# Dfam-consortium/RepeatAfterMe

Measured on AMD Instinct MI355X. Metric: flank_bp_aligned_per_sec (extension columns/s x flanks), higher is better.
Workload: dtype int32

## Files before the change

repeatafterme_amd/csrc/ramx_device.hip:

```cpp

#include <rccl/rccl.h>
#include <errno.h>
#include <fcntl.h>
#include <limits.h>
#include <sys/mman.h>
#include <unistd.h>
#include <stdarg.h>
#include <stdio.h>
#include <stdlib.h>
#include <string.h>
#include <time.h>
#include <algorithm>
#include <memory>
#include <vector>

#include "ramx_kernels_common.h"
#include "ramx_kernels_stream.h"
#include "ramx_kernels_resident.h"
#include "ramx_cp_api.h"
#include "ramx_pk_api.h"
#include "ramx_profile_api.h"
#include "ramx_align_api.h"
#include "ramx_pileup_api.h"
#include "ramx_dinuc_api.h"
// ... 774 lines not shown

static int direction_route(ramx_dev *d, const KArgs &a, int L, DirRoute *out)
{
  const RouteEnv e = route_env();
  DirRoute rt = route_gates(e, a.W, a.go, a.ge, a.tab, L, d->Nx, d->pk_r0, d->cp_flanks_ok != 0, d->trace_cb != NULL || d->verbose_cb != NULL,
                            dev_is_multi(d), d->peer_ready != 0, d->nranks, d->force_chain != 0, d->cus);
  const int W = a.W, tiles = d->Np / 64;
  if (rt.int32_can)
  {
    const int rc = (W == 14) ? prk_plan<14>(tiles, d->cus, &rt.block, &rt.blocks) : (W == 20) ? prk_plan<20>(tiles, d->cus, &rt.block, &rt.blocks) :
                   (W == 40) ? prk_plan<40>(tiles, d->cus, &rt.block, &rt.blocks) : prk_plan<80>(tiles, d->cus, &rt.block, &rt.blocks);
    if (rc != RAMX_OK) return rc;
  }
  if (rt.pk && ramx_pk_shape(W, tiles, &rt.pk_block, &rt.pk_blocks) != RAMX_OK) { ramx_set_error("packed-row kernel: occupancy query failed"); return RAMX_ERR_HIP; }
  route_settle(rt, e, d->Nx);
  *out = rt;
  return RAMX_OK;
}

static int mailbox_clear(ramx_dev *d)
{
  if (!d->hostbox_host) HIPCHK(hipMemsetAsync(d->xbox, 0, sizeof(PeerBox), d->stream));
  HIPCHK(hipStreamSynchronize(d->stream));
  if (d->hostbox_host) { memset((void *)d->hostbox_host, 0, sizeof(PeerBox)); __sync_synchronize(); }
  return RAMX_OK;
}

static int mailbox_mirror(ramx_dev *d, PeerBox **mirror)
{
  *mirror = NULL;
  if (!d->hostbox_host) return RAMX_OK;
  if (!d->hostbox_mirror) HIPCHK(hipMalloc((void **)&d->hostbox_mirror, sizeof(PeerBox)));
  HIPCHK(hipMemsetAsync(d->hostbox_mirror, 0, sizeof(PeerBox), d->stream));
  *mirror = d->hostbox_mirror;
  return RAMX_OK;
}

static int read_launch_state(ramx_dev *d, RamxCtl c[2], unsigned *errw)
{
  unsigned long long ew = 0;
  HIPCHK(hipStreamSynchronize(d->stream));
  int rc = d2h_small(d, c, d->d_ctl, 2 * sizeof(RamxCtl));
  if (rc == RAMX_OK) rc = d2h_small(d, &ew, d->d_err, sizeof(ew));
  *errw = (unsigned)ew;
  return rc;
}

#ifdef RAMX_PRK_TIMING
static int prk_timing_report(ramx_dev *d, unsigned long long *dbgbuf, size_t nw, bool pk, int block, int blocks, int L, int pk_r0)
{
  HIPCHK(hipStreamSynchronize(d->stream));
  unsigned long long *h = (unsigned long long *)malloc(nw * 8 * sizeof(unsigned long long));
  HIPCHK(hipMemcpy(h, dbgbuf, nw * 8 * sizeof(unsigned long long), hipMemcpyDeviceToHost));
  static const char *nm[6] = { "wait vote", "block barrier 1", "band", pk ? "early arrival" : "reduce+barrier 2", pk ? "late arrival" : "issue atomics", "loop top" };
  const int wpb = block / 64;
  fprintf(stderr, "PRK_TIMING %s blocks %d x %d threads, L %d, first row %d (ns per column)\n", pk ? "packed rows" : "int32 rows", blocks, block, L, pk ? pk_r0 : 0);
  for (int k = 0; k < 6; k++)
  {
    double s0 = 0, sO = 0, mx = 0, mn = 1e30;
    for (size_t i = 0; i < nw; i++)
    {
      const double v = 10.0 * (double)h[i * 8 + k] / L;
      if ((int)(i % wpb) == 0) s0 += v; else sO += v;
      if (v > mx) mx = v;
      if (v < mn) mn = v;
    }
    fprintf(stderr, "PRK_TIMING %-18s wave0 avg %8.1f  other waves avg %8.1f  min %8.1f  max %8.1f\n", nm[k], s0 / blocks,
            wpb > 1 ? sO / (double)(nw - blocks) : 0.0, mn, mx);
  }
  fprintf(stderr, "PRK_TIMING band by wave index:");
  for (int wv = 0; wv < wpb; wv++)
  {
    double sw = 0;
    for (int b = 0; b < blocks - 1; b++) sw += 10.0 * (double)h[((size_t)b * wpb + wv) * 8 + 2] / L;
    fprintf(stderr, " w%d %.0f", wv, sw / (blocks > 1 ? blocks - 1 : 1));
  }
  fprintf(stderr, "\n");
  {
    int gb = 0;
    for (int b = 1; b < blocks; b++) if (h[(size_t)b * wpb * 8 + 0] < h[(size_t)gb * wpb * 8 + 0]) gb = b;
    fprintf(stderr, "PRK_TIMING workgroup %d (shortest vote wait), per wave: wait vote | barrier | band | early | late | top\n", gb);
    for (int wv = 0; wv < wpb; wv++)
    {
      const unsigned long long *q = h + ((size_t)gb * wpb + wv) * 8;
      fprintf(stderr, "PRK_TIMING   w%d %7.0f %7.0f %7.0f %7.0f %7.0f %7.0f   rows full %llu lean %llu\n", wv, 10.0 * q[0] / L, 10.0 * q[1] / L, 10.0 * q[2] / L,
              10.0 * q[3] / L, 10.0 * q[4] / L, 10.0 * q[5] / L, q[6], q[7]);
    }
  }
  {
    const double half = L - L / 2;
    size_t never = 0, always = 0, wg_any = 0;
    double lanes = 0, cols = 0;
    int hist[6] = { 0, 0, 0, 0, 0, 0 };
    for (int b = 0; b < blocks; b++)
    {
      bool any = false;
      for (int wv = 0; wv < wpb; wv++)
      {
        const size_t i = (size_t)b * wpb + wv;
        const double c = (double)h[i * 8 + 6], l = (double)h[i * 8 + 7];
        if (c == 0) { never++; continue; }
        any = any || c > 0.5 * half;
        if (c > 0.9 * half) always++;
        lanes += l; cols += c;
        const double avg = l / c;
        hist[avg <= 1 ? 0 : avg <= 2 ? 1 : avg <= 4 ? 2 : avg <= 8 ? 3 : avg <= 16 ? 4 : 5]++;
      }
      if (any) wg_any++;
    }
    fprintf(stderr, "PRK_LEANSTAT second half (%.0f columns): %zu of %zu waves always LEAN, %zu non-LEAN in > 90 %% of the columns; workgroups with a wave "
            "non-LEAN in > 50 %%: %zu of %d; lanes per non-LEAN wave-column %.2f; waves by that average <=1: %d <=2: %d <=4: %d <=8: %d <=16: %d more: %d\n",
            half, never, nw, always, wg_any, blocks, cols > 0 ? lanes / cols : 0.0, hist[0], hist[1], hist[2], hist[3], hist[4], hist[5]);
  }
  free(h);
  (void)hipFree(dbgbuf);
  return RAMX_OK;
}

static int fam_timing_report(const unsigned long long *dbg)
{
  unsigned long long h[64];
  HIPCHK(hipMemcpy(h, dbg, sizeof(h), hipMemcpyDeviceToHost));
  static const char *nm[6] = { "vote + stop rule", "winner table+barrier", "band + contrib", "wave reduce", "end barrier", "loop top" };
  const double cols = h[6] ? (double)h[6] : 1.0;
  fprintf(stderr, "FAM_TIMING family 0 (block 0), %.0f columns, ns per column per wave:\n", cols);
  for (int k = 0; k < 6; k++)
    fprintf(stderr, "FAM_TIMING %-22s w0 %7.1f  w1 %7.1f  w2 %7.1f  w3 %7.1f\n", nm[k], 10.0 * h[k] / cols, 10.0 * h[8 + k] / cols,
            10.0 * h[16 + k] / cols, 10.0 * h[24 + k] / cols);
  return RAMX_OK;
}
#endif

#ifdef RAMX_CP_TIMING
static int cp_family_timing_report(const unsigned long long *dbg)
{
  unsigned long long h[16 * 16 + 8];
  HIPCHK(hipMemcpy(h, dbg, sizeof(h), hipMemcpyDeviceToHost));
  static const char *nm[12] = { "vote read + stop rule", "(after speculative band)", "row update", "reductions", "records/slide/window",
                                "sum+atomics+barrier", "-", "loop top", "wait: drain", "wait: samples + polling", "wait: fold",
                                "wait: LDS + barrier" };
  const double cols = h[16 * 16] ? (double)h[16 * 16] : 1.0;
  fprintf(stderr, "CP_TIMING block 0, %.0f columns, shader clocks per column (waves 0, 1, last two):\n", cols);
  int nw = 0;
  for (int w = 0; w < 16; w++) if (h[w * 16 + 0]) nw = w + 1;
  for (int k = 0; k < 12; k++)
    if (k == 6) fprintf(stderr, "CP_TIMING mispredicted columns: %.0f of %.0f\n", (double)h[6], cols);
    else fprintf(stderr, "CP_TIMING %-24s w0 %7.1f  w1 %7.1f  w%d %7.1f  w%d %7.1f\n", nm[k], h[k] / cols, h[16 + k] / cols,
                        nw > 1 ? nw - 2 : 0, h[(nw > 1 ? nw - 2 : 0) * 16 + k] / cols, nw > 0 ? nw - 1 : 0, h[(nw > 0 ? nw - 1 : 0) * 16 + k] / cols);
  return RAMX_OK;
}
#endif

static int prk_run(ramx_dev *d, const KArgs &a, int L, DirRoute &rt, bool *used)
{
  *used = false;
  const int W = a.W;
  const bool multi = rt.multi;
  int rc;
  if (multi)
  {
    int cannot = rt.int32_can ? 0 : 1;
    if ((rc = host_allreduce_flag(d, &cannot)) != RAMX_OK) return rc;
    rt.int32_can = !cannot;
  }
  const bool pk = rt.pk;
  const int pk_r0 = rt.pk_r0, pk_block = rt.pk_block, pk_blocks = rt.pk_blocks;
  int block = rt.block, blocks = rt.blocks;
// ... 18 lines not shown
  }
  memcpy(pa.tab, a.tab, sizeof(pa.tab));
  pa.pack_ok = getenv("RAMX_NO_FASTPACK") ? 0 : fast_pack_ok(pa.tab, a.go, a.ge, L, W);
  if (pa.pack_ok && getenv("RAMX_NO_MASKHI") == NULL) pa.pack_ok = 2;
  pa.lean_p = lean_p_of(pa.tab, a.go, a.ge);
  { const char *lm = getenv("RAMX_LEADER_MAX"); pa.leader_max = lm ? atoi(lm) : 3; if (pa.leader_max < 0) pa.leader_max = 0; if (pa.leader_max > 64) pa.leader_max = 64; }
  PKArgs ka;
  memset(&ka, 0, sizeof(ka));
  ka.spread = rt.spread; ka.rebase = rt.rebase;
  if (!pk && (rc = pack_rest(d)) != RAMX_OK) return rc;
  HIPCHK(hipMemsetAsync(d->d_vote, 0, PRK_NSETS * NSHARD * sizeof(PShard), d->stream));
  HIPCHK(hipMemsetAsync(d->d_err, 0, 64, d->stream));
  long long *sums_next = d->d_sums + (size_t)NSHARD * 4;
  const bool head = !pk || pk_r0 > 0;
  if (pk && pk_r0 > 0) { pa.L = pk_r0; pa.sums_next = sums_next; }
#ifdef RAMX_PRK_TIMING
  const size_t nw = pk ? (size_t)pk_blocks * (pk_block / 64) : (size_t)blocks * (block / 64);
  unsigned long long *dbgbuf = NULL;
  HIPCHK(hipMalloc((void **)&dbgbuf, nw * 8 * sizeof(unsigned long long)));
  HIPCHK(hipMemset(dbgbuf, 0, nw * 8 * sizeof(unsigned long long)));
  if (pk) ka.dbg = dbgbuf; else pa.dbg = dbgbuf;
#endif
  rc = RAMX_OK;
  const bool tmarks = getenv("RAMX_TIMING") != NULL;
  const double tm0 = now_ms();
  rt_mark("persistent route, memsets");
  if (head)
  {
    if (block == 256)
      rc = (W == 14) ? prk_launch<14, 256>(d, pa, blocks) : (W == 20) ? prk_launch<20, 256>(d, pa, blocks) :
           (W == 40) ? prk_launch<40, 256>(d, pa, blocks) : prk_launch<80, 256>(d, pa, blocks);
    else
      rc = (W == 14) ? prk_launch<14, 512>(d, pa, blocks) : (W == 20) ? prk_launch<20, 512>(d, pa, blocks) : prk_launch<40, 512>(d, pa, blocks);
  }
  rt_mark("first rows launched (int32 kernel)");
  if (rc == RAMX_OK && pk)
  {
    ka.S = d->d_state[0]; ka.bases = d->d_bases; ka.bounds = d->d_bounds; ka.trim = d->d_trim;
    ka.vote = d->d_vote; ka.cons_out = d->d_cons; ka.err = d->d_err;
    ka.peers = pa.peers; ka.box = pa.box; ka.mirror = pa.mirror; ka.rank = pa.rank; ka.nranks = pa.nranks;
    ka.xblock = 0;
    if (ka.nranks > 1 && getenv("RAMX_NO_PK_EXCHANGER") == NULL)
    {
      int cap = 0;
      if (ramx_pk_capacity(W, pk_block, &cap) == RAMX_OK && pk_blocks + 1 <= cap) ka.xblock = pk_blocks;
    }
    ka.Np = d->Np; ka.Nx = d->Nx; ka.L = L; ka.go = a.go; ka.ge = a.ge; ka.cap = a.cap; ka.minimp = a.minimp;
    ka.when_to_stop = a.when_to_stop; ka.nblocks = pk_blocks;
    memcpy(ka.tab, a.tab, sizeof(ka.tab));
    ka.lean_p = pa.lean_p; ka.leader_max = pa.leader_max;
    ka.spec_on = getenv("RAMX_NO_PK_SPEC") == NULL ? 1 : 0;
    { const char *we = getenv("RAMX_TEST_PK_WRONG_EVERY"); ka.test_wrong_every = we ? atoi(we) : 0; }
    { const char *ck = getenv("RAMX_PK_CKPT"); const int v = ck ? atoi(ck) : 0; ka.ckpt = (v == 1 || v == 2 || v == 4 || v == 8) ? v : 0; }
    { const char *ts = getenv("RAMX_TEST_PK_SPREAD"); if (ts) ka.spread = atoi(ts); }
    ka.spread_rows = ka.spread;
    { const char *ts = getenv("RAMX_TEST_PK_SPREAD_ROWS"); if (ts) ka.spread_rows = atoi(ts); }
    d->last_packed_r0 = pk_r0;
    const int seg = pk_segment_columns(L, a.when_to_stop);
    const int NWw = (2 * W + 1 + 8) / 8 + 2;
    long long *sbuf[2] = { d->d_sums + (size_t)NSHARD * 4, d->d_sums + (size_t)2 * NSHARD * 4 };
    const long long *sums_in = pk_r0 > 0 ? sbuf[0] : d->d_sums;
    int nextbuf = pk_r0 > 0 ? 1 : 0;
    int ctl_i = 0;
    auto words_for = [&](int r_end) { int wn = ((r_end + 7) >> 3) + NWw + 2; return wn < d->KW ? wn : d->KW; };
    if (ka.nranks > 1 && !head) test_delay_rank(d);
    for (int r = pk_r0, s_i = 0; r < L && rc == RAMX_OK; s_i++)
    {
      const int r1 = seg > 0 ? std::min(L, (r / seg + 1) * seg) : L;
      if ((rc = pack_settle(d)) != RAMX_OK) return rc;
      if (d->packed_kw < words_for(r1))
      {
        if ((rc = launch_pack(d, d->Nx, d->Np, W, d->packed_kw, words_for(r1), d->stream)) != RAMX_OK) break;
        d->packed_kw = words_for(r1);
      }
      HIPCHK(hipMemsetAsync(d->d_vote, 0, PRK_NSETS * NSHARD * sizeof(PShard), d->stream));
      ka.r0 = r; ka.Lseg = r1; ka.sums_in = sums_in;
      ka.sums_next = r1 < L ? sbuf[nextbuf] : NULL;
      if (r1 < L) HIPCHK(hipMemsetAsync(sbuf[nextbuf], 0, (size_t)NSHARD * 4 * sizeof(long long), d->stream));
      ka.ctl_in = d->d_ctl + ctl_i; ka.ctl_out = d->d_ctl + (ctl_i ^ 1);
      if (r == 0) ka.ctl_out = d->d_ctl;
      const double tm1 = now_ms();
      rc = ramx_pk_launch(d->stream, W, pk_block, pk_blocks, ka);
      if (rc != RAMX_OK) { ramx_set_error("packed-row kernel: launch failed (W %d, %d workgroups of %d threads)", W, pk_blocks, pk_block); break; }
      if (tmarks) fprintf(stderr, "RAMX_TIMING       run: piece %d (rows %d..%d, %d x %d threads) launched %.3f ms after the first launch (launch call %.3f ms)\n", s_i, r, r1, pk_blocks, pk_block, now_ms() - tm0, now_ms() - tm1);
      const int out_i = (r == 0) ? 0 : (ctl_i ^ 1);
      if (r1 >= L) break;
      const int r2 = std::min(L, (r1 / seg + 1) * seg);
      if (d->packed_kw < words_for(r2))
      {
        if ((rc = launch_pack(d, d->Nx, d->Np, W, d->packed_kw, words_for(r2), d->pack_stream)) != RAMX_OK) break;
        HIPCHK(hipEventRecord(d->pack_done, d->pack_stream));
        d->pack_busy = 1;
        d->packed_kw = words_for(r2);
      }
      RamxCtl c2[2];
      unsigned errw = 0;
      HIPCHK(hipStreamSynchronize(d->stream));
      if (tmarks) fprintf(stderr, "RAMX_TIMING       run: piece %d complete %.3f ms after the first launch\n", s_i, now_ms() - tm0);
      if ((rc = read_launch_state(d, c2, &errw)) != RAMX_OK) break;
      rt_mark("piece: control block and error word read");
      const RamxCtl &hc = c2[out_i];
      if (hc.stopped || hc.pad != 0 || errw != 0 || hc.rows_done < r1) break;
      sums_in = sbuf[nextbuf]; nextbuf ^= 1; ctl_i = out_i; r = r1;
    }
    if (pk) { block = pk_block; blocks = pk_blocks; }
  }
// ... 2317 lines not shown
```

repeatafterme_amd/csrc/ramx_kernels_packed.h:

```cpp
#pragma once

#include "ramx_kernels_vote.h"
#include "ramx_pk_api.h"

template <int W>
struct PkCfg
{
  static constexpr int B = 2 * W + 1, NP = W + 1, NW = (B + 8) / 8 + 2, NG = (B + 31) / 32, Q = W + 1;
};

#define PKB_NEG2 ((int)0x80008000u)
#ifndef PKB_GROUP
#define PKB_GROUP 2
#endif
#ifndef PKB_PT
#define PKB_PT 2
#endif

__device__ __forceinline__ int pkb_add_sat(int a, int b) { return pk_i(__builtin_elementwise_add_sat(pk_v(a), pk_v(b))); }
__device__ __forceinline__ int pkb_sub_sat(int a, int b) { return pk_i(__builtin_elementwise_sub_sat(pk_v(a), pk_v(b))); }
__device__ __forceinline__ int pkb_max(int a, int b) { return pk_i(__builtin_elementwise_max(pk_v(a), pk_v(b))); }
__device__ __forceinline__ void pkb_add_to_hi(int &dst, int a, int b) { asm("v_add_i16 %0, %1, %2 op_sel:[0,0,1] clamp" : "+v"(dst) : "v"(a), "v"(b)); }
__device__ __forceinline__ int pkb_add_lo(int a, int b) { int d; asm("v_add_i16 %0, %1, %2 clamp" : "=v"(d) : "v"(a), "v"(b)); return d; }
__device__ __forceinline__ int pkb_hmax(int p) { const pk_s2 q = pk_v(p); return q.x > q.y ? (int)q.x : (int)q.y; }
__device__ __forceinline__ unsigned pkb_lds_off(const void *p) { return (unsigned)(size_t)(__attribute__((address_space(3))) const void *)p; }

__device__ __forceinline__ unsigned pkb_mask_word(unsigned wv, int kb, int bdy9x4 )
{
  int s = bdy9x4 - 32 * kb;
  s = s < 0 ? 0 : s;
  const unsigned m = s >= 32 ? 0u : (0xffffffffu << s);
  return wv | m;
}

struct PkTabs
{
  int4 t4[4][256];
  int tp[4][256];
};

template <int BLOCK>
__device__ __forceinline__ void pkb_tabs_init(PkTabs &pt, const int (&tab)[RAMX_NCLASS][4])
{
  for (int i = threadIdx.x; i < 256; i += BLOCK)
  {
    const int hi = i >> 4, lo = (i & 15) ^ ((hi & 3) << 2);
    int q[4];
#pragma unroll
    for (int c = 0; c < 4; c++)
    {
      const int sl = lo < RAMX_NCLASS ? tab[lo][c] : (lo == 15 ? -32768 : 0);
      const int sh = hi < RAMX_NCLASS ? tab[hi][c] : (hi == 15 ? -32768 : 0);
      q[c] = (sl & 0xffff) | (sh << 16);
      pt.tp[c][i] = q[c];
    }
#pragma unroll
    for (int wv = 0; wv < 4; wv++) pt.t4[wv][i] = make_int4(q[wv], q[(wv + 1) & 3], q[(wv + 2) & 3], q[(wv + 3) & 3]);
  }
}

template <int W, int BLOCK, bool FULL>
__device__ __forceinline__ void pkb_band(const int go2, const int ge2, const PkTabs &pt, const int wsel, const int ph4, const unsigned (&w)[PkCfg<W>::NW],
                                         int (&R)[PkCfg<W>::NP], int (&E)[PkCfg<W>::NP], int &best, int (&kg)[PkCfg<W>::NG], int (&bA)[4], int &maxE)
{
// ... 143 lines not shown
    if (hit[h]) jb = 64 * h + __builtin_ctzll(hit[h]);
  if (lane == leader)
  {
#pragma unroll
    for (int c = 0; c < 4; c++) bestA[c] = best[c];
    jbest = jb;
  }
}

template <class A>
__device__ __forceinline__ int pkb_stop_rule(const A &a, const int r, const long long (&v)[4], const int fl, int *st, const int lane)
{
  long long mx = ((long long)__builtin_amdgcn_readfirstlane(st[1]) << 32) | (long long)(unsigned)__builtin_amdgcn_readfirstlane(st[0]);
  int mr = __builtin_amdgcn_readfirstlane(st[2]), ov = __builtin_amdgcn_readfirstlane(st[3]);
  long long cw = 0;
  int bw = 0;
#pragma unroll
  for (int k = 0; k < 4; k++)
  {
    const long long vk = ((long long)__builtin_amdgcn_readfirstlane((int)(v[k] >> 32)) << 32) |
                         (long long)(unsigned)__builtin_amdgcn_readfirstlane((int)v[k]);
    if (vk > 2147483647LL || vk < -2147483648LL) ov = 1;
    if (vk > cw) { cw = vk; bw = k; }
  }
  int dist = mr - r;
  dist = dist < 0 ? -dist : dist;
  const int nm = cw >= mx + (long long)dist * a.minimp ? 1 : 0;
  if (nm && !fl) { mr = r; mx = cw; }
  int d2 = r - mr;
  d2 = d2 < 0 ? -d2 : d2;
  const int stp = d2 >= a.when_to_stop ? 1 : 0;
  if (lane == 0) { st[0] = (int)mx; st[1] = (int)(mx >> 32); st[2] = mr; st[3] = ov; }
  return bw | (nm << 2) | (stp << 3) | (fl << 4);
}

#ifdef RAMX_PRK_TIMING
#ifdef RAMX_PRK_TIMING_TAIL
#define PKB_TICK_ON (2 * r >= a.L)
#else
#define PKB_TICK_ON true
#endif
#define PKB_TICK(k) do { const unsigned long long t_ = wall_clock64(); if (PKB_TICK_ON) tsum[k] += t_ - tlast; tlast = t_; } while (0)
#else
#define PKB_TICK(k) do { } while (0)
#endif

template <int W, int BLOCK>
__global__ __launch_bounds__(BLOCK, BLOCK / 256) void ramx_packed_kernel(const PKArgs a)
{
  constexpr int NP = PkCfg<W>::NP, NW = PkCfg<W>::NW, NG = PkCfg<W>::NG, Q = PkCfg<W>::Q, WPB = BLOCK / 64;
  constexpr bool VW = (BLOCK % 256) != 0;
  constexpr int BW = VW ? WPB - 1 : WPB, VOTER = VW ? BW : 0;
  constexpr bool SPEC = W <= 40;
  struct Smem
  {
    PkTabs pt;
    long long tot[2][2][4];
    int word[2][2];
    int cnt[2][2];
    int st[4];
    int lead[WPB][2 * NP + NW + 1];
    int eb[SPEC ? BLOCK * NP : 1];
  };
  __shared__ __attribute__((aligned(16))) Smem sm;
  const int lane = threadIdx.x & 63, wave = threadIdx.x >> 6;
  const int tile = blockIdx.x * BW + wave;
  const bool live = wave < BW && tile < (a.Np >> 6);
  const int n = (live ? tile : 0) * 64 + lane;
  int4 *S = a.S + (size_t)(live ? tile : 0) * Q * 64 + lane;
  const int2 bd = a.bounds[n];
  const int bdy = (n >= a.Nx) ? 0x3fffffff : (bd.x > bd.y ? -0x40000000 : bd.y);
#define PKB_BDY9X4(b) ((b) > 0x07ffffff ? 0x3fffffff : ((b) < -0x08000000 ? -0x40000000 : 4 * ((b) + 9)))
  const int shard = blockIdx.x % NSHARD;
  const int go2 = pk_two(a.go), ge2 = pk_two(a.ge);

  pkb_tabs_init<BLOCK>(sm.pt, a.tab);
  if (threadIdx.x < 16) (&sm.tot[0][0][0])[threadIdx.x] = 0;
  if (threadIdx.x < 4) (&sm.cnt[0][0])[threadIdx.x] = 0;
  if (threadIdx.x < 4) (&sm.word[0][0])[threadIdx.x] = 0;

  long long max_ext = 0;
  int max_row = -1, rows_done = a.r0, ovf = 0, stopped = 0, failed = 0, carried = 0;
  if (a.r0 > 0)
  {
    const RamxCtl *cp = a.ctl_in;
    const long long me = cp->max_ext;
    max_ext = ((long long)__builtin_amdgcn_readfirstlane((int)(me >> 32)) << 32) | (long long)(unsigned)__builtin_amdgcn_readfirstlane((int)me);
    max_row = __builtin_amdgcn_readfirstlane(cp->max_row);
    rows_done = __builtin_amdgcn_readfirstlane(cp->rows_done);
    ovf = __builtin_amdgcn_readfirstlane(cp->overflow);
    stopped = (__builtin_amdgcn_readfirstlane(cp->stopped) || rows_done < a.r0) ? 1 : 0;
    const int cpad = __builtin_amdgcn_readfirstlane(cp->pad);
    failed = cpad;
    carried = __builtin_amdgcn_readfirstlane(cp->besta);
  }
  else if (live) a.trim[n] = make_int2(0, 0);
  stopped = __builtin_amdgcn_readfirstlane(stopped); max_row = __builtin_amdgcn_readfirstlane(max_row);
  rows_done = __builtin_amdgcn_readfirstlane(rows_done); carried = __builtin_amdgcn_readfirstlane(carried);
  const bool skip = stopped || failed || a.r0 >= a.Lseg;
  if (threadIdx.x == 0) { sm.st[0] = (int)max_ext; sm.st[1] = (int)(max_ext >> 32); sm.st[2] = max_row; sm.st[3] = ovf; }

  if (blockIdx.x == a.nblocks)
  {
    if (wave != 0 || stopped || failed || a.r0 >= a.Lseg) return;
    for (int r = a.r0; r < a.Lseg; r++)
    {
      PShard *vb = a.vote;
      asm volatile("" : "+s"(vb));
      long long v[4];
      prk_wait_vote(a, vb, a.sums_in, r == a.r0 ? (a.r0 == 0 ? 1 : 2) : 0, r, lane, (a.nblocks - (lane & (NSHARD - 1)) + NSHARD - 1) / NSHARD, failed, v, true);
      const int fl = __any(failed) ? 1 : 0;
      const int dword = pkb_stop_rule(a, r, v, fl, sm.st, lane);
      if (fl) { if (lane == 0) __hip_atomic_fetch_max(a.err, 1u, __ATOMIC_RELAXED, __HIP_MEMORY_SCOPE_AGENT); break; }
      if (lane == 0) a.cons_out[r] = (signed char)(dword & 3);
      if (lane < NSHARD)
      {
        PShard *z = vb + (size_t)((r + 3) & (PRK_NSETS - 1)) * NSHARD + lane;
#pragma unroll
        for (int k = 0; k < 4; k++) __hip_atomic_store(&z->word[k], 0ULL, __ATOMIC_RELAXED, __HIP_MEMORY_SCOPE_AGENT);
      }
      if ((dword & 8) || r == a.L - 1) break;
    }
    return;
  }

  int R[NP], E[NP];
  int high, pos, pbase = 0;
  {
    const int jcut = bdy - (a.r0 - 1);
    int bmax = -2147483647 - 1, bmin = 2147483647;
    const int4 *S1 = S;
    asm volatile("" : "+v"(S1));
// ... 22 lines not shown
    auto rel16 = [&](int x, bool inb) __attribute__((always_inline)) -> int
    {
      int d = x - pbase;
      d = d < -32768 ? -32768 : (d > 32767 ? 32767 : d);
      return inb ? d : -32768;
    };
    int eprev = -32768;
    static_for([&](auto qc) __attribute__((always_inline))
    {
      constexpr int q = decltype(qc)::value;
      if constexpr ((q & 7) == 0) __builtin_amdgcn_sched_barrier(0);
      const int4 v = S2[(size_t)q * 64];
      const bool in0 = 2 * q <= jcut2, in1 = q < W && 2 * q + 1 <= jcut2;
      const int m0 = rel16(v.x, in0), e0 = rel16(v.y, in0);
      const int m1 = q < W ? rel16(v.z, in1) : -32768, e1 = q < W ? rel16(v.w, in1) : -32768;
      R[q] = (m0 & 0xffff) | (m1 << 16);
      E[q] = (eprev & 0xffff) | (e0 << 16);
      eprev = e1;
      if constexpr (q == W) { high = v.z; pos = v.w; }
    }, std::make_integer_sequence<int, Q>{});
    __builtin_amdgcn_sched_barrier(0);
  }
  if (skip)
  {
    if (blockIdx.x == 0 && threadIdx.x == 0)
    {
      RamxCtl o;
      o.max_ext = max_ext; o.max_row = max_row; o.stopped = stopped; o.rows_done = rows_done; o.overflow = ovf; o.besta = carried; o.pad = failed;
      *a.ctl_out = o;
    }
    return;
  }

  unsigned w[NW], wnext;
  {
    const int k0 = (a.r0 + 8) >> 3;
    const unsigned *bp = a.bases + (size_t)k0 * a.Np + n;
    static_for([&](auto kc) __attribute__((always_inline)) { constexpr int k = decltype(kc)::value; w[k] = pkb_mask_word(bp[(size_t)k * a.Np], k0 + k, PKB_BDY9X4(bdy)); },
               std::make_integer_sequence<int, NW>{});
    wnext = bp[(size_t)NW * a.Np];
  }
  __syncthreads();

  int prevBest = 0x3fffffff;
  int full_rows = 0, lean_rows = 0, wrong_rows = 0;
#ifdef RAMX_PRK_TIMING
  unsigned long long tsum[6] = { 0, 0, 0, 0, 0, 0 }, tlast = wall_clock64();
#endif
  int Rb[SPEC ? NP : 1], high_b = 0, pos_b = 0, prev_b = 0, pbase_b = 0;
  int ck_row = 0, ck_valid = 0, ck_calm = 64;
  unsigned ck_log = 0;
  int replay_to = -1, pend = 0;
  int spec = 0, guess = 0;
  for (int r = a.r0; r < a.Lseg; r++)
  {
    PKB_TICK(5);
    PShard *vb = a.vote;
    asm volatile("" : "+s"(vb));
    if (((r + 8) & 7) == 0 && r > a.r0 && replay_to < 0)
    {
      static_for([&](auto kc) __attribute__((always_inline)) { constexpr int k = decltype(kc)::value; w[k] = w[k + 1]; }, std::make_integer_sequence<int, NW - 1>{});
      const int kn = ((r + 8) >> 3) + NW;
      int nn = n, bb = bdy;
      asm volatile("" : "+v"(nn), "+v"(bb));
      w[NW - 1] = pkb_mask_word(wnext, kn - 1, PKB_BDY9X4(bb));
      wnext = a.bases[(size_t)kn * a.Np + nn];
      if (ck_row != r) ck_valid = 0;
    }
    const int par = r & 1, npar = (r + 1) & 1;
    const bool hand_over = r == a.Lseg - 1 && a.Lseg < a.L;
    int besta = 0, next_guess = 0;
    long long dgw = 0;
    bool new_max = false, last_col = false;

    auto decide = [&]() __attribute__((always_inline)) -> bool
    {
      if (wave == VOTER)
      {
        long long v[4];
        int lv = lane;
        asm volatile("" : "+v"(lv));
        prk_wait_vote(a, vb, a.sums_in, r == a.r0 ? (a.r0 == 0 ? 1 : 2) : 0, r, lv, (a.nblocks - (lv & (NSHARD - 1)) + NSHARD - 1) / NSHARD, failed, v, blockIdx.x == a.xblock);
        const int fl = __any(failed) ? 1 : 0;
        const int dword = pkb_stop_rule(a, r, v, fl, sm.st, lane);
        const int bw = dword & 3;
        if (lane == 0)
        {
          sm.word[par][0] = dword;
          if (fl) __hip_atomic_fetch_max(a.err, 1u, __ATOMIC_RELAXED, __HIP_MEMORY_SCOPE_AGENT);
        }
        if (blockIdx.x == a.xblock && !fl)
        {
          if (lane == 0) a.cons_out[r] = (signed char)bw;
          if (lane < NSHARD)
          {
            PShard *z = vb + (size_t)((r + 3) & (PRK_NSETS - 1)) * NSHARD + lane;
#pragma unroll
            for (int k = 0; k < 4; k++) __hip_atomic_store(&z->word[k], 0ULL, __ATOMIC_RELAXED, __HIP_MEMORY_SCOPE_AGENT);
          }
        }
      }
      PKB_TICK(0);
      asm volatile("s_waitcnt lgkmcnt(0)\n\ts_barrier" ::: "memory");
      PKB_TICK(1);
      int dw, gw;
      asm volatile("ds_read_b64 %0, %1\n\ts_waitcnt lgkmcnt(0)" : "=v"(dgw) : "v"(pkb_lds_off(&sm.word[par][0])) : "memory");
      dw = __builtin_amdgcn_readfirstlane((int)dgw); gw = __builtin_amdgcn_readfirstlane((int)(dgw >> 32));
      next_guess = gw;
      if (dw & 16) { failed = 1; return false; }
      besta = dw & 3;
      new_max = (dw & 4) != 0;
      stopped = (dw >> 3) & 1;
      rows_done = r + 1;
      last_col = stopped || r == a.L - 1;
      return true;
    };

    auto arrive = [&](const int set, const long long t0, const long long t1, const long long t2, const long long t3) __attribute__((always_inline))
    {
      const long long mine = lane == 0 ? t0 : lane == 1 ? t1 : lane == 2 ? t2 : t3;
      int old = 0;
      if (lane < 4) asm volatile("ds_add_u64 %0, %1" : : "v"(pkb_lds_off(&sm.tot[set][npar][lane])), "v"(mine) : "memory");
      if (lane == 0) asm volatile("ds_add_rtn_u32 %0, %1, %2\n\ts_waitcnt lgkmcnt(0)" : "=v"(old) : "v"(pkb_lds_off(&sm.cnt[set][npar])), "v"(1) : "memory");
      old = __builtin_amdgcn_readfirstlane(old);
      if (old == WPB - 1)
      {
        long long t = 0;
        if (lane < 4)
        {
          asm volatile("ds_read_b64 %0, %1\n\ts_waitcnt lgkmcnt(0)" : "=v"(t) : "v"(pkb_lds_off(&sm.tot[set][npar][lane])) : "memory");
          if (set == 1)
          {
            asm volatile("ds_write_b64 %0, %1" : : "v"(pkb_lds_off(&sm.tot[set][npar][lane])), "v"(0LL) : "memory");
            if (hand_over)
            {
              int lq = lane;
              asm volatile("" : "+v"(lq));
              __hip_atomic_fetch_add(&a.sums_next[shard * 4 + lq], t, __ATOMIC_RELAXED, __HIP_MEMORY_SCOPE_AGENT);
            }
            else
            {
              PShard *sh = vb + (size_t)((r + 1) & (PRK_NSETS - 1)) * NSHARD + shard;
              __hip_atomic_fetch_add(&sh->word[lane], (unsigned long long)t + PRK_BIAS + PRK_TICKET, __ATOMIC_RELAXED, __HIP_MEMORY_SCOPE_AGENT);
            }
          }
        }
        if (set == 1 && lane == 0) asm volatile("ds_write_b32 %0, %1" : : "v"(pkb_lds_off(&sm.cnt[set][npar])), "v"(0) : "memory");
        if constexpr (SPEC)
        {
          const long long q0 = prk_readlane_u64((unsigned long long)t, 0), q1 = prk_readlane_u64((unsigned long long)t, 1);
          const long long q2 = prk_readlane_u64((unsigned long long)t, 2), q3 = prk_readlane_u64((unsigned long long)t, 3);
          long long c = 0;
          int g = 0;
          if (q0 > c) { c = q0; g = 0; }
          if (q1 > c) { c = q1; g = 1; }
          if (q2 > c) { c = q2; g = 2; }
          if (q3 > c) { c = q3; g = 3; }
          const int informative = !(q0 == q1 && q1 == q2 && q2 == q3) && a.spec_on;
          if (lane == 0) sm.word[par][1] = (informative << 8) | g;
        }
      }
    };

    int *myEb = sm.eb + (SPEC ? threadIdx.x * NP : 0);
    bool pass_spec = false;
    int wsel = 0;
    const bool silent = r < replay_to;
    if (silent) wsel = (int)((ck_log >> (2 * ((r - ck_row) & 7))) & 3u);
    else if (r == replay_to)
    {
      besta = pend & 3; new_max = (pend & 4) != 0; last_col = (pend & 8) != 0;
      wsel = besta;
      replay_to = -1;
    }
    else if (spec)
    {
      pass_spec = true;
      wsel = guess;
      if (a.test_wrong_every > 0 && (r % a.test_wrong_every) == 0) wsel = (guess + 1) & 3;
    }
    else
    {
      if (!decide()) break;
      wsel = besta;
    }
    bool confirmed_arrival = false;
    bool gave_up = false;
    bool rewind = false;
    do
    {
      const int set = pass_spec ? 0 : 1;
      const int jhi = bdy - r;
      const int capfloor = (high + a.cap) > 0 ? (high + a.cap) : 0;
      bool lean = false, early = false;
      unsigned long long leaders = 0;
      if (live && a.lean_p >= 0)
      {
        const unsigned long long keep = __ballot((n < a.Nx) && !((prevBest + 2 * a.lean_p <= capfloor) && (prevBest + a.lean_p <= high)));
        if (keep == 0) { lean = true; early = true; }
        else if (__popcll(keep) <= a.leader_max) { lean = true; leaders = keep; }
      }
      if (!live) early = true;
      const bool send = !silent && (pass_spec || !last_col);
      if (early && send)
      {
        const long long t = wave_sum_nonneg31((live && n < a.Nx) ? capfloor : 0);
        arrive(set, t, t, t, t);
      }
      PKB_TICK(3);
      if (__builtin_amdgcn_readfirstlane(early ? 1 : 0) == 0) __builtin_amdgcn_s_setprio(2);

      int contrib[4] = { 0, 0, 0, 0 };
      if (live)
      {
        const int ph4 = 4 * ((r + 8) & 7);
        int best, kg[NG], bA[4], maxE;
        if (lean) pkb_band<W, BLOCK, false>(go2, ge2, sm.pt, wsel, ph4, w, R, E, best, kg, bA, maxE);
        else pkb_band<W, BLOCK, true>(go2, ge2, sm.pt, wsel, ph4, w, R, E, best, kg, bA, maxE);
        int rel, jbest = 0, bestA[4] = { NEG, NEG, NEG, NEG };
        if (lean) rel = pkb_hmax(best);
        else
        {
          int bkey = kg[NG - 1], bg = NG - 1;
          rel = kg[NG - 1] >> 16;
#pragma unroll
          for (int g = NG - 2; g >= 0; g--)
          {
            const int v = kg[g] >> 16;
            const bool take = v >= rel;
            rel = take ? v : rel;
            bkey = take ? kg[g] : bkey;
            bg = take ? g : bg;
          }
          jbest = 32 * bg + 31 - (bkey & 31);
          const int mE = pkb_hmax(maxE);
          int rot[4];
#pragma unroll
          for (int i = 0; i < 4; i++) rot[i] = jhi < 1 ? NEG : pbase + imax(pkb_hmax(bA[i]), mE);
#pragma unroll
          for (int c = 0; c < 4; c++)
          {
            const int i = (c - wsel) & 3;
            bestA[c] = i == 0 ? rot[0] : i == 1 ? rot[1] : i == 2 ? rot[2] : rot[3];
          }
        }
        const int bestF = jhi < 0 ? SENT : pbase + rel;
        for (unsigned long long rest = leaders; rest != 0; rest &= rest - 1)
          pkb_leader_rows<W, BLOCK>(sm.pt, sm.lead[wave], (r + 8) & 7, __builtin_ctzll(rest), pbase, jhi, bestF, w, R, E, bestA, jbest);
        if ((r & 63) == 63)
        {
          int mn = 0x7fff7fff, jj = jhi;
          asm volatile("" : "+v"(jj));
          static_for([&](auto kc) __attribute__((always_inline))
          {
            constexpr int k = decltype(kc)::value;
// ... 3 lines not shown
            v = 2 * k <= jj ? v : 0x7fff7fff;
            mn = pk_i(__builtin_elementwise_min(pk_v(mn), pk_v(v)));
          }, std::make_integer_sequence<int, NP>{});
          const pk_s2 q = pk_v(mn);
          const int lowest = q.x < q.y ? (int)q.x : (int)q.y;
          if (n < a.Nx && jhi >= 0 && (rel - lowest > a.spread_rows || rel > RAMX_PK_LIMIT || lowest < -RAMX_PK_LIMIT))
            __hip_atomic_fetch_max(a.err, 2u, __ATOMIC_RELAXED, __HIP_MEMORY_SCOPE_AGENT);
        }
        if ((r & 15) == 15 && __any(jhi >= 0 && (rel > a.rebase || rel < -a.rebase)))
        {
          const int mv = jhi >= 0 ? rel : 0;
          const int bb = pk_two(mv);
          static_for([&](auto kc) __attribute__((always_inline)) { constexpr int k = decltype(kc)::value; R[k] = pkb_sub_sat(R[k], bb); E[k] = pkb_sub_sat(E[k], bb); },
                     std::make_integer_sequence<int, NP>{});
          pbase += mv;
        }
        prevBest = bestF;
        if (bestF > high) { high = bestF; pos = r + jbest - W; }
        if (n < a.Nx)
        {
          const int capv = high + a.cap;
#pragma unroll
          for (int c = 0; c < 4; c++)
          {
            const int b = bestA[c] < 0 ? 0 : bestA[c];
            contrib[c] = (b >= capv) ? b : capv;
          }
        }
        if (!pass_spec && !silent) { if (lean) lean_rows++; else full_rows++; }
      }
      PKB_TICK(2);
      if (!early && send)
      {
#ifndef PKB_PROBE_NO_REDUCE
        long long t[4];
#ifndef PKB_PROBE_OLD_REDUCE
        wave_sum4_nonneg31(contrib, t);
#else
#pragma unroll
        for (int c = 0; c < 4; c++) t[c] = wave_sum_nonneg31(contrib[c]);
#endif
        const long long t0 = t[0], t1 = t[1], t2 = t[2], t3 = t[3];
#else
        const long long t0 = __builtin_amdgcn_readfirstlane(contrib[0]), t1 = __builtin_amdgcn_readfirstlane(contrib[1]);
        const long long t2 = __builtin_amdgcn_readfirstlane(contrib[2]), t3 = __builtin_amdgcn_readfirstlane(contrib[3]);
#endif
        arrive(set, t0, t1, t2, t3);
      }
      PKB_TICK(4);
      __builtin_amdgcn_s_setprio(0);
      if (!pass_spec) { confirmed_arrival = send; break; }
      if (!decide()) { gave_up = true; break; }
      const bool right = besta == wsel;
      if (wave == VOTER)
      {
        if (lane < 4)
        {
          long long t;
          asm volatile("ds_read_b64 %0, %1\n\ts_waitcnt lgkmcnt(0)" : "=v"(t) : "v"(pkb_lds_off(&sm.tot[0][npar][lane])) : "memory");
          asm volatile("ds_write_b64 %0, %1" : : "v"(pkb_lds_off(&sm.tot[0][npar][lane])), "v"(0LL) : "memory");
          if (right && !last_col)
          {
            if (hand_over)
            {
              int lq = lane;
              asm volatile("" : "+v"(lq));
              __hip_atomic_fetch_add(&a.sums_next[shard * 4 + lq], t, __ATOMIC_RELAXED, __HIP_MEMORY_SCOPE_AGENT);
            }
            else
            {
              PShard *sh = vb + (size_t)((r + 1) & (PRK_NSETS - 1)) * NSHARD + shard;
              __hip_atomic_fetch_add(&sh->word[lane], (unsigned long long)t + PRK_BIAS + PRK_TICKET, __ATOMIC_RELAXED, __HIP_MEMORY_SCOPE_AGENT);
            }
          }
        }
        if (lane == 0) asm volatile("ds_write_b32 %0, %1" : : "v"(pkb_lds_off(&sm.cnt[0][npar])), "v"(0) : "memory");
      }
      if (right) break;
      if constexpr (SPEC)
      {
        if (live)
        static_for([&](auto kc) __attribute__((always_inline)) { constexpr int k = decltype(kc)::value; R[k] = Rb[k]; E[k] = myEb[k]; }, std::make_integer_sequence<int, NP>{});
        high = high_b; pos = pos_b; prevBest = prev_b; pbase = pbase_b;
        ck_calm = 0;
        pend = besta | (new_max ? 4 : 0) | (last_col ? 8 : 0);
        replay_to = r;
        r = ck_row - 1;
        rewind = true;
      }
      wrong_rows++;
    } while (false);
    if (gave_up) break;
    if (rewind || silent) continue;
    if constexpr (SPEC)
    {
      ck_log |= (unsigned)besta << (2 * ((r - ck_row) & 7));
      ck_calm = ck_calm < 64 ? ck_calm + 1 : 64;
    }
#ifndef PKB_PROBE_NO_TRIM
    if (new_max && live)
#else
    if (new_max && live && r < 0)
#endif
    {
      int nn = n;
      asm volatile("" : "+v"(nn));
      a.trim[nn] = make_int2(high, pos);
    }
    if (last_col || hand_over) break;
    if constexpr (SPEC)
    {
      if (confirmed_arrival)
      {
        asm volatile("s_waitcnt lgkmcnt(0)\n\ts_barrier" ::: "memory");
        int gw;
        asm volatile("ds_read_b32 %0, %1\n\ts_waitcnt lgkmcnt(0)" : "=v"(gw) : "v"(pkb_lds_off(&sm.word[par][1])) : "memory");
        next_guess = __builtin_amdgcn_readfirstlane(gw);
      }
      spec = next_guess >> 8; guess = next_guess & 3;
      if (spec)
      {
        const int dist = a.ckpt > 0 ? a.ckpt : ck_calm < 32 ? 1 : ck_calm < 40 ? 2 : ck_calm < 48 ? 4 : 8;
        if (!ck_valid || ((r + 1) & (dist - 1)) == 0)
        {
#ifndef PKB_PROBE_NO_BACKUP
          if (live)
          static_for([&](auto kc) __attribute__((always_inline)) { constexpr int k = decltype(kc)::value; Rb[k] = R[k]; myEb[k] = E[k]; }, std::make_integer_sequence<int, NP>{});
#else
          Rb[0] = R[0];
#endif
          high_b = high; pos_b = pos; prev_b = prevBest; pbase_b = pbase;
          ck_row = r + 1; ck_valid = 1; ck_log = 0;
        }
      }
    }
  }
#ifdef RAMX_PRK_TIMING
  if (a.dbg != NULL && (threadIdx.x & 63) == 0)
  {
#pragma unroll
    for (int k = 0; k < 6; k++) a.dbg[((size_t)blockIdx.x * WPB + wave) * 8 + k] += tsum[k];
    a.dbg[((size_t)blockIdx.x * WPB + wave) * 8 + 6] += (unsigned long long)full_rows;
    a.dbg[((size_t)blockIdx.x * WPB + wave) * 8 + 7] += (unsigned long long)lean_rows;
  }
#endif

  if (live && rows_done > a.r0)
  {
    int bz = bdy;
    asm volatile("" : "+v"(bz));
    const int rl = rows_done - 1, jh = bz - rl;
    const int edge = rl < W ? a.go + (rl + 1) * a.ge : SENT;
    int tid = threadIdx.x;
    asm volatile("" : "+v"(tid));
    int4 *S3 = a.S + (size_t)(blockIdx.x * BW + (tid >> 6)) * Q * 64 + (tid & 63);
    auto val = [&](int half, int j, bool is_e) __attribute__((always_inline)) -> int
    {
      if (j > jh) { const int f = j < W ? edge : SENT; return is_e ? f + a.ge : f; }
      return pbase + half;
    };
    static_for([&](auto qc) __attribute__((always_inline))
    {
      constexpr int q = decltype(qc)::value;
      const int m0 = val((int)(short)R[q], 2 * q, false), e0 = val(E[q] >> 16, 2 * q, true);
      if constexpr (q < W)
      {
        const int m1 = val(R[q] >> 16, 2 * q + 1, false), e1 = val((int)(short)E[q + 1 < NP ? q + 1 : 0], 2 * q + 1, true);
        S3[(size_t)q * 64] = make_int4(m0, e0, m1, e1);
      }
      else S3[(size_t)q * 64] = make_int4(m0, e0, high, pos);
    }, std::make_integer_sequence<int, Q>{});
  }
  if (blockIdx.x == 0 && threadIdx.x == 0)
  {
    RamxCtl o;
    o.max_ext = ((long long)sm.st[1] << 32) | (long long)(unsigned)sm.st[0]; o.max_row = sm.st[2]; o.stopped = stopped; o.rows_done = rows_done;
    o.overflow = sm.st[3];
    o.besta = ((carried & 0xffff) + lean_rows) | ((((carried >> 16) & 0xffff) + wrong_rows) << 16);
    o.pad = failed;
    *a.ctl_out = o;
  }
}
```

repeatafterme_amd/csrc/ramx_pk_api.h:

```cpp
#pragma once

#include <hip/hip_runtime.h>

#include "ramx_kernels_common.h"

struct PShard;
struct PeerBox;

struct PKArgs
{
  int4 *S;
  const unsigned *bases;
  const int2 *bounds;
  int2 *trim;
  const long long *sums_in;
  PShard *vote;
  const RamxCtl *ctl_in;
  RamxCtl *ctl_out;
  signed char *cons_out;
  unsigned *err;
  PeerBox *const *peers;
  PeerBox *box;
  PeerBox *mirror;
  int rank, nranks;
  int xblock;
  long long *sums_next;
  int Np, Nx, r0, Lseg, L, go, ge, cap, minimp, when_to_stop, nblocks;
  int tab[RAMX_NCLASS][4];
  int lean_p;
  int leader_max;
  int spread;
  int spread_rows;
  int rebase;
  int spec_on;
  int test_wrong_every;
  int ckpt;
  unsigned long long *dbg;
};

#define RAMX_PK_LIMIT 32000

int ramx_pk_plan(int W, int go, int ge, const int (&tab)[RAMX_NCLASS][4], int *spread, int *rebase);
int ramx_pk_capacity(int W, int block, int *cap);
int ramx_pk_shape(int W, int tiles, int *block, int *blocks);
int ramx_pk_launch(hipStream_t st, int W, int block, int blocks, const PKArgs &a);
```

Before: 18.71 billion.

## Move packed-kernel vote duty to a wave that arrived early each column

In the speculative packed-row kernel, when no dedicated voter wave exists, the vote/decide duty no longer stays fixed on wave 0. Each wave writes a byte flag to LDS saying whether it was late. The next column picks the first wave that was not late as voter, so the reduction work lands on a wave that would otherwise idle at the barrier. This adds an LDS byte write per wave and widens the shared-word read to 128 bits, and it makes the voter a runtime value instead of a compile-time constant. Environment variables can pin the voter, and timing instrumentation counts the columns where the duty moved.

```diff
diff --git a/repeatafterme_amd/csrc/ramx_device.hip b/repeatafterme_amd/csrc/ramx_device.hip
--- a/repeatafterme_amd/csrc/ramx_device.hip
+++ b/repeatafterme_amd/csrc/ramx_device.hip
@@ -850,15 +850,22 @@
   HIPCHK(hipStreamSynchronize(d->stream));
   unsigned long long *h = (unsigned long long *)malloc(nw * 8 * sizeof(unsigned long long));
   HIPCHK(hipMemcpy(h, dbgbuf, nw * 8 * sizeof(unsigned long long), hipMemcpyDeviceToHost));
+  unsigned long long *moved = (unsigned long long *)calloc(nw, sizeof(unsigned long long));
+  if (pk) for (size_t i = 0; i < nw; i++) { moved[i] = h[i * 8 + 6] >> 32; h[i * 8 + 6] &= 0xffffffffULL; }
+#ifdef RAMX_PRK_TIMING_TAIL
+  const double ncol = pk ? (double)(L - (L + 1) / 2 > 0 ? L - (L + 1) / 2 : 1) : (double)L;
+#else
+  const double ncol = (double)L;
+#endif
   static const char *nm[6] = { "wait vote", "block barrier 1", "band", pk ? "early arrival" : "reduce+barrier 2", pk ? "late arrival" : "issue atomics", "loop top" };
   const int wpb = block / 64;
-  fprintf(stderr, "PRK_TIMING %s blocks %d x %d threads, L %d, first row %d (ns per column)\n", pk ? "packed rows" : "int32 rows", blocks, block, L, pk ? pk_r0 : 0);
+  fprintf(stderr, "PRK_TIMING %s blocks %d x %d threads, L %d, first row %d (ns per column, %.0f columns accounted)\n", pk ? "packed rows" : "int32 rows", blocks, block, L, pk ? pk_r0 : 0, ncol);
   for (int k = 0; k < 6; k++)
   {
     double s0 = 0, sO = 0, mx = 0, mn = 1e30;
     for (size_t i = 0; i < nw; i++)
     {
-      const double v = 10.0 * (double)h[i * 8 + k] / L;
+      const double v = 10.0 * (double)h[i * 8 + k] / ncol;
       if ((int)(i % wpb) == 0) s0 += v; else sO += v;
       if (v > mx) mx = v;
       if (v < mn) mn = v;
@@ -870,7 +877,7 @@
   for (int wv = 0; wv < wpb; wv++)
   {
     double sw = 0;
-    for (int b = 0; b < blocks - 1; b++) sw += 10.0 * (double)h[((size_t)b * wpb + wv) * 8 + 2] / L;
+    for (int b = 0; b < blocks - 1; b++) sw += 10.0 * (double)h[((size_t)b * wpb + wv) * 8 + 2] / ncol;
     fprintf(stderr, " w%d %.0f", wv, sw / (blocks > 1 ? blocks - 1 : 1));
   }
   fprintf(stderr, "\n");
@@ -881,8 +888,15 @@
     for (int wv = 0; wv < wpb; wv++)
     {
       const unsigned long long *q = h + ((size_t)gb * wpb + wv) * 8;
-      fprintf(stderr, "PRK_TIMING   w%d %7.0f %7.0f %7.0f %7.0f %7.0f %7.0f   rows full %llu lean %llu\n", wv, 10.0 * q[0] / L, 10.0 * q[1] / L, 10.0 * q[2] / L,
-              10.0 * q[3] / L, 10.0 * q[4] / L, 10.0 * q[5] / L, q[6], q[7]);
+      fprintf(stderr, "PRK_TIMING   w%d %7.0f %7.0f %7.0f %7.0f %7.0f %7.0f   rows full %llu lean %llu\n", wv, 10.0 * q[0] / ncol, 10.0 * q[1] / ncol, 10.0 * q[2] / ncol,
+              10.0 * q[3] / ncol, 10.0 * q[4] / ncol, 10.0 * q[5] / ncol, q[6], q[7]);
+    }
+    if (pk)
+    {
+      unsigned long long all = 0, most = 0;
+      for (int b = 0; b < blocks; b++) { const unsigned long long m = moved[(size_t)b * wpb]; all += m; if (m > most) most = m; }
+      fprintf(stderr, "PRK_TIMING columns with the vote duty off wave 0: workgroup %d %llu, average %.1f, most %llu (of %d)\n", gb, moved[(size_t)gb * wpb],
+              (double)all / blocks, most, L - pk_r0);
     }
   }
   {
@@ -911,6 +925,7 @@
             half, never, nw, always, wg_any, blocks, cols > 0 ? lanes / cols : 0.0, hist[0], hist[1], hist[2], hist[3], hist[4], hist[5]);
   }
   free(h);
+  free(moved);
   (void)hipFree(dbgbuf);
   return RAMX_OK;
 }
@@ -1035,6 +1050,8 @@
     ka.spec_on = getenv("RAMX_NO_PK_SPEC") == NULL ? 1 : 0;
     { const char *we = getenv("RAMX_TEST_PK_WRONG_EVERY"); ka.test_wrong_every = we ? atoi(we) : 0; }
     { const char *ck = getenv("RAMX_PK_CKPT"); const int v = ck ? atoi(ck) : 0; ka.ckpt = (v == 1 || v == 2 || v == 4 || v == 8) ? v : 0; }
+    ka.voter_pin = getenv("RAMX_PK_FIXED_VOTER") != NULL && atoi(getenv("RAMX_PK_FIXED_VOTER")) == 1 ? 0 : -1;
+    { const char *tv = getenv("RAMX_TEST_PK_VOTER"); if (tv && atoi(tv) >= 0 && atoi(tv) < pk_block / 64) ka.voter_pin = atoi(tv); }
     { const char *ts = getenv("RAMX_TEST_PK_SPREAD"); if (ts) ka.spread = atoi(ts); }
     ka.spread_rows = ka.spread;
     { const char *ts = getenv("RAMX_TEST_PK_SPREAD_ROWS"); if (ts) ka.spread_rows = atoi(ts); }
diff --git a/repeatafterme_amd/csrc/ramx_kernels_packed.h b/repeatafterme_amd/csrc/ramx_kernels_packed.h
--- a/repeatafterme_amd/csrc/ramx_kernels_packed.h
+++ b/repeatafterme_amd/csrc/ramx_kernels_packed.h
@@ -10,6 +10,7 @@
 };
 
 #define PKB_NEG2 ((int)0x80008000u)
+typedef int pk_i4 __attribute__((ext_vector_type(4)));
 #ifndef PKB_GROUP
 #define PKB_GROUP 2
 #endif
@@ -259,11 +260,12 @@
   constexpr bool VW = (BLOCK % 256) != 0;
   constexpr int BW = VW ? WPB - 1 : WPB, VOTER = VW ? BW : 0;
   constexpr bool SPEC = W <= 40;
+  constexpr bool MOVE = SPEC && !VW;
   struct Smem
   {
     PkTabs pt;
     long long tot[2][2][4];
-    int word[2][2];
+    int word[2][MOVE ? 4 : 2];
     int cnt[2][2];
     int st[4];
     int lead[WPB][2 * NP + NW + 1];
@@ -284,7 +286,7 @@
   pkb_tabs_init<BLOCK>(sm.pt, a.tab);
   if (threadIdx.x < 16) (&sm.tot[0][0][0])[threadIdx.x] = 0;
   if (threadIdx.x < 4) (&sm.cnt[0][0])[threadIdx.x] = 0;
-  if (threadIdx.x < 4) (&sm.word[0][0])[threadIdx.x] = 0;
+  if (threadIdx.x < (MOVE ? 8 : 4)) (&sm.word[0][0])[threadIdx.x] = 0;
 
   long long max_ext = 0;
   int max_row = -1, rows_done = a.r0, ovf = 0, stopped = 0, failed = 0, carried = 0;
@@ -413,6 +415,11 @@
   unsigned ck_log = 0;
   int replay_to = -1, pend = 0;
   int spec = 0, guess = 0;
+  int voter = MOVE ? (a.voter_pin > 0 ? a.voter_pin : 0) : VOTER;
+  int late_lo = 0, late_hi = 0;
+#ifdef RAMX_PRK_TIMING
+  int moved_cols = 0;
+#endif
   for (int r = a.r0; r < a.Lseg; r++)
   {
     PKB_TICK(5);
@@ -436,7 +443,7 @@
 
     auto decide = [&]() __attribute__((always_inline)) -> bool
     {
-      if (wave == VOTER)
+      if (wave == (MOVE ? voter : VOTER))
       {
         long long v[4];
         int lv = lane;
@@ -465,8 +472,18 @@
       asm volatile("s_waitcnt lgkmcnt(0)\n\ts_barrier" ::: "memory");
       PKB_TICK(1);
       int dw, gw;
-      asm volatile("ds_read_b64 %0, %1\n\ts_waitcnt lgkmcnt(0)" : "=v"(dgw) : "v"(pkb_lds_off(&sm.word[par][0])) : "memory");
-      dw = __builtin_amdgcn_readfirstlane((int)dgw); gw = __builtin_amdgcn_readfirstlane((int)(dgw >> 32));
+      if constexpr (MOVE)
+      {
+        pk_i4 q;
+        asm volatile("ds_read_b128 %0, %1\n\ts_waitcnt lgkmcnt(0)" : "=v"(q) : "v"(pkb_lds_off(&sm.word[par][0])) : "memory");
+        dw = __builtin_amdgcn_readfirstlane(q.x); gw = __builtin_amdgcn_readfirstlane(q.y);
+        late_lo = __builtin_amdgcn_readfirstlane(q.z); late_hi = __builtin_amdgcn_readfirstlane(q.w);
+      }
+      else
+      {
+        asm volatile("ds_read_b64 %0, %1\n\ts_waitcnt lgkmcnt(0)" : "=v"(dgw) : "v"(pkb_lds_off(&sm.word[par][0])) : "memory");
+        dw = __builtin_amdgcn_readfirstlane((int)dgw); gw = __builtin_amdgcn_readfirstlane((int)(dgw >> 32));
+      }
       next_guess = gw;
       if (dw & 16) { failed = 1; return false; }
       besta = dw & 3;
@@ -562,6 +579,11 @@
         else if (__popcll(keep) <= a.leader_max) { lean = true; leaders = keep; }
       }
       if (!live) early = true;
+      if constexpr (MOVE)
+      {
+        if (!silent && lane == 0)
+          asm volatile("ds_write_b8 %0, %1" : : "v"(pkb_lds_off(reinterpret_cast<const char *>(&sm.word[par][2]) + wave)), "v"(early ? 0 : (1 << (wave & 3))) : "memory");
+      }
       const bool send = !silent && (pass_spec || !last_col);
       if (early && send)
       {
@@ -671,7 +693,7 @@
       if (!pass_spec) { confirmed_arrival = send; break; }
       if (!decide()) { gave_up = true; break; }
       const bool right = besta == wsel;
-      if (wave == VOTER)
+      if (wave == (MOVE ? voter : VOTER))
       {
         if (lane < 4)
         {
@@ -732,11 +754,33 @@
       if (confirmed_arrival)
       {
         asm volatile("s_waitcnt lgkmcnt(0)\n\ts_barrier" ::: "memory");
-        int gw;
-        asm volatile("ds_read_b32 %0, %1\n\ts_waitcnt lgkmcnt(0)" : "=v"(gw) : "v"(pkb_lds_off(&sm.word[par][1])) : "memory");
-        next_guess = __builtin_amdgcn_readfirstlane(gw);
+        if constexpr (MOVE)
+        {
+          pk_i4 q;
+          asm volatile("ds_read_b128 %0, %1\n\ts_waitcnt lgkmcnt(0)" : "=v"(q) : "v"(pkb_lds_off(&sm.word[par][0])) : "memory");
+          next_guess = __builtin_amdgcn_readfirstlane(q.y);
+          late_lo = __builtin_amdgcn_readfirstlane(q.z); late_hi = __builtin_amdgcn_readfirstlane(q.w);
+        }
+        else
+        {
+          int gw;
+          asm volatile("ds_read_b32 %0, %1\n\ts_waitcnt lgkmcnt(0)" : "=v"(gw) : "v"(pkb_lds_off(&sm.word[par][1])) : "memory");
+          next_guess = __builtin_amdgcn_readfirstlane(gw);
+        }
       }
       spec = next_guess >> 8; guess = next_guess & 3;
+      if constexpr (MOVE)
+      {
+#ifdef RAMX_PRK_TIMING
+        if (voter != 0) moved_cols++;
+#endif
+        if (a.voter_pin < 0)
+        {
+          unsigned y = (unsigned)(late_lo | late_hi);
+          y |= y >> 16; y |= y >> 8; y &= 15u;
+          voter = y == 15u ? 0 : __builtin_ctz(~y);
+        }
+      }
       if (spec)
       {
         const int dist = a.ckpt > 0 ? a.ckpt : ck_calm < 32 ? 1 : ck_calm < 40 ? 2 : ck_calm < 48 ? 4 : 8;
@@ -759,7 +803,7 @@
   {
 #pragma unroll
     for (int k = 0; k < 6; k++) a.dbg[((size_t)blockIdx.x * WPB + wave) * 8 + k] += tsum[k];
-    a.dbg[((size_t)blockIdx.x * WPB + wave) * 8 + 6] += (unsigned long long)full_rows;
+    a.dbg[((size_t)blockIdx.x * WPB + wave) * 8 + 6] += (unsigned long long)full_rows | ((unsigned long long)moved_cols << 32);
     a.dbg[((size_t)blockIdx.x * WPB + wave) * 8 + 7] += (unsigned long long)lean_rows;
   }
 #endif
diff --git a/repeatafterme_amd/csrc/ramx_pk_api.h b/repeatafterme_amd/csrc/ramx_pk_api.h
--- a/repeatafterme_amd/csrc/ramx_pk_api.h
+++ b/repeatafterme_amd/csrc/ramx_pk_api.h
@@ -35,6 +35,7 @@
   int spec_on;
   int test_wrong_every;
   int ckpt;
+  int voter_pin;
   unsigned long long *dbg;
 };
 
```

Measured after the change: 18.83 billion, median of 6. About the same (+0.6%).
